# bjzhb666/GS-LoRA

Measured on AMD Instinct MI355X. Metric: forgetting-step images/sec, ViT-P8S8 d6 112px r=8, higher is better.
Workload: dtype fp16

## Files before the change

### gs-lora_amd/gslora_hip/_lib.py

```python
import ctypes as C
import os

import contextlib

_HERE = os.path.dirname(os.path.abspath(__file__))
LIB_PATH = os.environ.get("GSLORA_HIP_LIB") or os.path.join(_HERE, "libgslora_hip.so")
DEV_LIB_PATH = os.path.join(_HERE, "libgslora_hip_dev.so")

F32, BF16, F16 = 0, 1, 2
EPI_STORE, EPI_BIAS_RES_F32, EPI_BIAS_GELU, EPI_MUL, EPI_PATCH, EPI_STORE_F32, EPI_STORE_QKV_HM, EPI_BIAS_RES_BF16, EPI_PATCH_BF16 = 0, 1, 2, 3, 4, 5, 6, 7, 8
EPI_MUL_G8, EPI_BIAS_GELU_G8, EPI_BIAS_RES_F16, EPI_PATCH_F16, EPI_STORE_LN, EPI_STORE_QKV_HM_LN = 9, 10, 11, 12, 13, 14
VERIF_FLIP_SUM, VERIF_PLAIN = 0, 1
U8_NCHW, U8_NHWC = 0, 1
NORM_SPLIT = 8
SEED_ON_DEVICE = 0x80000000

_vp, _i, _l, _f, _d, _u64, _u32 = C.c_void_p, C.c_int, C.c_long, C.c_float, C.c_double, C.c_uint64, C.c_uint32

SIGNATURES = {
    "gsl_version": [],
    "gsl_last_error": [],
    "gsl_patchify": [_vp, _vp, _i, _i, _i, _i, _i, _i, _vp],
    "gsl_unfold_patches": [_vp, _vp, _i, _i, _i, _i, _i, _i, _i, _i, _i, _vp],
    "gsl_patchify_u8": [_vp, _i, _vp, _vp, _i, _i, _i, _i, _i, _i, _vp],
    "gsl_unfold_patches_u8": [_vp, _i, _vp, _vp, _i, _i, _i, _i, _i, _i, _i, _i, _i, _vp],
    "gsl_gemm_nt": [_vp, _i, _vp, _i, _i, _vp, _i, _vp, _i, _i, _i, _i, _i, _i, _f, _vp, _vp, _vp, _vp, _vp, _i,
                    _vp, _vp, _i, _f, _u64, _u32, _vp],
    "gsl_gemm_nt_lora": [_vp, _i, _vp, _i, _i, _vp, _i, _vp, _i, _f, _vp, _i, _i, _i, _i, _i, _vp, _vp, _vp, _vp, _vp, _i,
                         _f, _u64, _u32, _vp],
    "gsl_gemm_mulgrad_ws_elems": [_i, _i, _i],
    "gsl_gemm_nt_lora_mulgrad": [_vp, _i, _vp, _i, _i, _vp, _i, _vp, _i, _f, _vp, _i, _i, _i, _vp, _vp, _i,
                                 _vp, _i, _vp, _l, _l, _vp, _vp, _l, _l, _i, _i, _vp, _i, _f, _i, _vp, _vp],
    "gsl_layernorm_fwd": [_vp, _l, _vp, _vp, _f, _vp, _vp, _vp, _i, _i, _i, _i, _vp],
    "gsl_layernorm_fwd_lora": [_vp, _l, _vp, _vp, _f, _vp, _vp, _vp, _i, _i, _vp, _i, _f, _vp, _vp],
    "gsl_layernorm_bwd": [_vp, _vp, _l, _vp, _vp, _vp, _vp, _vp, _l, _vp, _i, _i, _i, _i, _i, _f, _u64, _u32, _l, _i, _vp, _vp],
    "gsl_attention_fwd": [_vp, _vp, _vp, _i, _i, _i, _f, _i, _i, _vp],
    "gsl_attention_bwd": [_vp, _vp, _vp, _vp, _vp, _vp, _i, _i, _i, _f, _i, _i, _vp],
    "gsl_attention_fwd_cls": [_vp, _vp, _vp, _vp, _i, _i, _i, _f, _i, _i, _vp],
    "gsl_attention_bwd_cls": [_vp, _vp, _vp, _vp, _vp, _vp, _vp, _i, _i, _i, _f, _i, _i, _i, _vp],
    "gsl_lora_grad_ws_elems": [_i, _i, _i],
    "gsl_lora_grad": [_vp, _l, _vp, _i, _vp, _l, _l, _i, _i, _i, _i, _i, _vp, _vp, _vp],
    "gsl_lora_grad_batch_ws_elems": [_vp, _i],
    "gsl_lora_grad_batch": [_vp, _i, _vp, _i, _vp, _vp],
    "gsl_cosface_prep": [_vp, _vp, _i, _i, _vp],
    "gsl_head_fwd": [_vp, _i, _i, _vp, _vp, _f, _vp, _vp, _vp, _vp, _vp, _vp, _i, _i, _i, _f, _f, _vp, _i, _i, _vp],
    "gsl_head_bwd": [_vp, _vp, _vp, _i, _i, _vp, _vp, _vp, _vp, _vp, _vp, _vp, _i, _i, _i, _f, _i, _i, _f, _u64, _u32, _i, _i, _i, _vp, _vp, _i, _vp],
    "gsl_head_fwd_margin": [_vp, _i, _i, _vp, _vp, _f, _vp, _vp, _vp, _vp, _vp, _vp, _i, _i, _i, _f, _f, _vp, _i, _i, _i, _d, _i, _vp, _vp],
    "gsl_head_bwd_margin": [_vp, _vp, _vp, _i, _i, _vp, _vp, _vp, _vp, _vp, _vp, _vp, _i, _i, _i, _f, _i, _i, _f, _u64, _u32, _i, _i, _i, _vp,
                            _vp, _i, _i, _d, _i, _vp, _vp, _vp],
    "gsl_ce_fwd": [_vp, _vp, _vp, _vp, _i, _i, _vp],
    "gsl_ce_bwd": [_vp, _vp, _vp, _f, _vp, _i, _i, _i, _vp],
    "gsl_proto_kl_fwd": [_vp, _vp, _vp, _vp, _vp, _i, _i, _i, _vp],
    "gsl_loss_combine": [_vp, _vp, _vp, _vp, _vp, _vp, _vp, _f, _f, _f, _f, _f, _f, _f, _f, _vp, _vp, _vp, _vp],
    "gsl_loss_combine_pack": [_vp, _vp, _i, _f, _f, _f, _f, _f, _f, _vp, _vp, _vp, _vp],
# ... 69 lines not shown
```

### gs-lora_amd/gslora_hip/build.py

```python
import os
import subprocess
import sys

HERE = os.path.dirname(os.path.abspath(__file__))
CSRC = os.path.join(os.path.dirname(HERE), "csrc")
SOURCES = ["gemm.hip", "norm.hip", "lora.hip", "head.hip", "attention.hip", "verif.hip"]
SOURCES_F16 = ["gemm.hip", "attention.hip"]
HEADERS = ["gsl_common.h", "gsl_h16.h", "exports.map", "gelu_g8_table.inc"]
DEV_ONLY = ["gemm_dev_a.inc", "gemm_dev_b.inc", "gemm_dev_c.inc", "gemm_w4.inc", "gemm_o4.inc"]
OUT = os.path.join(HERE, "libgslora_hip.so")
OUT_DEV = os.path.join(HERE, "libgslora_hip_dev.so")


def needs_build(dev=False):
    out = OUT_DEV if dev else OUT
    if not os.path.exists(out):
        return True
    t = os.path.getmtime(out)
    deps = [os.path.join(CSRC, s) for s in SOURCES + HEADERS + (DEV_ONLY if dev else [])]
    deps.append(os.path.join(os.path.dirname(os.path.dirname(HERE)), "include", "gslora_hip.h"))
    return any(os.path.getmtime(d) > t for d in deps)


def build(force=False, verbose=True, dev=False, defines=(), out=None, tag=None):
# ... 39 lines not shown
```

### gs-lora_amd/gslora_hip/ops.py

```python
import ctypes

import torch

from . import _lib as L

ATTN_MAX_T = 1025


def check_num_tokens(model, T):
    if T > ATTN_MAX_T:
        raise NotImplementedError(f"{model}: this geometry gives {T} tokens per image; the gs-lora_amd attention kernels take at most "
                                  f"{ATTN_MAX_T} (GSL_ATTN_MAX_T: a 32 x 32 patch grid plus the cls token)")


DT = {torch.float32: L.F32, torch.bfloat16: L.BF16, torch.float16: L.F16}


def _p(t):
    return None if t is None else t.data_ptr()


def _stream():
    return torch.cuda.current_stream().cuda_stream

# ... 282 lines not shown
                                           _stream()), "gsl_attention_fwd_cls")
    return o, lse


def attention_bwd_cls(qkv, o, d_o_cls, lse, B, T, H, scale, layout=0, q_cls=None):
    _need(qkv, o, d_o_cls, lse, q_cls)
    nw = 2 if layout == 2 else 3
    dqkv = torch.empty(B * T, nw * H * 64, device=qkv.device, dtype=qkv.dtype)
    dq = torch.empty(B, H * 64, device=qkv.device, dtype=qkv.dtype) if layout == 2 else None
    compact = o.shape[0] == B and lse.dim() == 2
    L.check(L.load().gsl_attention_bwd_cls(_p(qkv), _p(q_cls), _p(o), _p(d_o_cls), _p(lse), _p(dqkv), _p(dq), B, T, H, float(scale),
                                           code(qkv.dtype), int(layout), 1 if compact else 0, _stream()), "gsl_attention_bwd_cls")
    return (dqkv, dq) if layout == 2 else dqkv


_ws_cache = {}
_ws_retired = []


def lora_grad(Y, U, G, gsn, gsj, r, accumulate=True, gscale=None):
    if not (Y.is_cuda and U.is_cuda and Y.stride(1) == 1 and U.stride(1) == 1):
        raise RuntimeError("lora_grad: operands must be CUDA tensors with unit column stride")
    M, N = Y.shape
    lib = L.load()
    need = lib.gsl_lora_grad_ws_elems(M, N, r)
    key = (Y.device.index,)
    ws = _ws_cache.get(key)
    if ws is None or ws.numel() < need:
        if ws is not None:
            _ws_retired.append(ws)
# ... 329 lines not shown
```

### gs-lora_amd/gslora_hip/vit_runner.py

```python
import os

import torch

from . import _lib as L
from . import ops

PADK = 64
OP16 = (torch.bfloat16, torch.float16)
SITE_EMB = 1_000_000
GRAD_STREAM_BF16 = os.environ.get("GSLORA_GRAD_STREAM", "bf16").lower() != "f32"
FWD_STREAM = os.environ.get("GSLORA_FWD_STREAM", "f16").lower()
if FWD_STREAM not in ("f16", "bf16", "f32"):
    raise ValueError(f"GSLORA_FWD_STREAM must be f16, bf16 or f32, not {FWD_STREAM!r}")
GP8 = os.environ.get("GSLORA_GP8", "1") != "0"

FUSE_LORA_GRAD = True
TAIL_CLS = True
QSPLIT = True
INK_MIN_ROWS = 8192
LN1_FOLD = os.environ.get("GSLORA_LN1_FOLD", "1") != "0"
GRAD_TARGET_EXP = int(os.environ.get("GSLORA_GRAD_TARGET_EXP", "0"))
if GRAD_TARGET_EXP and not 4 <= GRAD_TARGET_EXP <= 15:
    raise ValueError(f"GSLORA_GRAD_TARGET_EXP={GRAD_TARGET_EXP}: 0 (default) or 4 .. 15")
INK_SMALL = True
LGRAD_BATCH_MAX_ROWS = 1 << 30
LN_LORA = False
QKV_HEAD_MAJOR = True


class BlockSpec:
    __slots__ = ("ln1", "qkv_w", "qkv_b", "out", "ln2", "l1", "l2", "qkv_lora")

    def __init__(self, ln1, qkv_w, qkv_b, out, ln2, l1, l2, qkv_lora=None):
# ... 173 lines not shown
            self._wcache[key] = ent
        return ent[1]

    def w_conv(self, name, param, dtype):
        def build(p):
            w2 = p.permute(0, 2, 3, 1).reshape(p.shape[0], -1).contiguous()
            return w2 if dtype == torch.float32 else ops.cast(w2, dtype)
        return self._cached(self._wcache, (name, "conv", dtype), param, build)

    def w_kpad(self, name, param, kpad, dtype):
        def build(p):
            w2 = torch.zeros(p.shape[0], kpad, device=p.device, dtype=torch.float32)
            w2[:, :p.shape[1]] = p
            return w2 if dtype == torch.float32 else ops.cast(w2, dtype)
        return self._cached(self._wcache, (name, "kpad", kpad, dtype), param, build)

    def wT(self, name, param, dtype):
        return self._cached(self._wcache, (name, "t", dtype), param, lambda p: ops.transpose_cast(p.contiguous(), dtype))

    PACK_GEOM = {
        "A_rows": lambda R, C, r: (C, 1, r, C, PADK, C),
        "B_cols": lambda R, C, r: (r, 1, R, r, R, PADK),
        "BT_rows": lambda R, C, r: (1, r, r, R, PADK, R),
        "AT_cols": lambda R, C, r: (1, C, C, r, C, PADK),
        "A_rows16": lambda R, C, r: (C, 1, r, C, 16, C),
        "B_cols32": lambda R, C, r: (r, 1, R, r, R, 32),
        "BT_rows16": lambda R, C, r: (1, r, r, R, 16, R),
        "AT_cols32": lambda R, C, r: (1, C, C, r, C, 32),
    }

# ... 150 lines not shown
            pw = self.w_conv("pe", sp.patch_w, dt) if sp.patch_is_conv else self.w("pe", sp.patch_w, dt)
        xbf = dt in OP16 and FWD_STREAM != "f32"
        xf16 = xbf and (FWD_STREAM == "f16" or dt == torch.float16)
        xdt = (torch.float16 if xf16 else torch.bfloat16) if xbf else torch.float32
        epi_res = (L.EPI_BIAS_RES_F16 if xf16 else L.EPI_BIAS_RES_BF16) if xbf else L.EPI_BIAS_RES_F32
        x = torch.empty(M, D, device=img.device, dtype=xdt)
        ops.gemm_nt(patches, pw, x, epilogue=(L.EPI_PATCH_F16 if xf16 else L.EPI_PATCH_BF16) if xbf else L.EPI_PATCH, bias=sp.patch_b.detach(),
                    pos=sp.pos.detach()[0, :T].contiguous(), cls=sp.cls.detach().reshape(-1), T=T,
                    p_drop=p_emb, seed=seed, site=SITE_EMB | sflag)
        del patches
        stash = []
        for i, blk in enumerate(sp.blocks):
            n1, n2 = blk.ln1, blk.ln2
            attn_lora_live = attn_site and not blk.qkv_lora.merged
            fold = LN1_FOLD and dt in OP16 and x.dtype == dt and not attn_lora_live
            if fold:
                mean1, rstd1 = ops.layernorm_stats(x, D, M, D, n1.weight.detach(), n1.bias.detach(), eps, dt)
                xn = None
            else:
                xn, mean1, rstd1 = ops.layernorm_fwd(x, D, M, D, n1.weight.detach(), n1.bias.detach(), eps, dt)
            tail = TAIL_CLS and i == len(sp.blocks) - 1 and sp.pool == "cls"
            qsplit = tail and QSPLIT and not attn_site
            inner = H * 64
            hm = 1 if (QKV_HEAD_MAJOR and dt in OP16) else 0
            epi_qkv = L.EPI_STORE_QKV_HM if hm else L.EPI_STORE
            uq = q_cls = None
            if qsplit and fold:
                wf, cq, dq_ = self.w_ln(f"qkv{i}", blk.qkv_w, n1.weight, n1.bias, blk.qkv_b, dt)
                qkv = torch.empty(M, 2 * inner, device=img.device, dtype=dt)
                ops.gemm_nt(x, wf[inner:], qkv, epilogue=L.EPI_STORE_LN, pos=mean1, cls=rstd1, aux=cq[inner:], bias=dq_[inner:])
                q_cls = torch.empty(B, inner, device=img.device, dtype=dt)
                ops.gemm_nt(x.view(B, T * D)[:, :D], wf[:inner], q_cls, epilogue=L.EPI_STORE_LN, T=T, pos=mean1, cls=rstd1,
                            aux=cq[:inner], bias=dq_[:inner])
                hm = 2
            elif qsplit:
                wq = self.w(f"qkv{i}", blk.qkv_w, dt)
                qb_ = None if blk.qkv_b is None else blk.qkv_b.detach()
                qkv = torch.empty(M, 2 * inner, device=img.device, dtype=dt)
                ops.gemm_nt(xn, wq[inner:], qkv, bias=None if qb_ is None else qb_[inner:])
                q_cls = torch.empty(B, inner, device=img.device, dtype=dt)
                ops.gemm_nt(xn.view(B, T * D)[:, :D], wq[:inner], q_cls, bias=None if qb_ is None else qb_[:inner].contiguous())
                hm = 2
# ... 2 lines not shown
                qo = self.qkv_lora_ops(i, blk.qkv_lora, dt)
                uq = torch.empty(M, PADK, device=img.device, dtype=dt)
                ops.gemm_nt(xn, qo["A_rows"], uq, alpha=s_lora)
                ops.gemm_nt(xn, self.w(f"qkv{i}", blk.qkv_w, dt), qkv, A2=uq, W2=qo["Bblk"], epilogue=epi_qkv, T=T,
                            bias=None if blk.qkv_b is None else blk.qkv_b.detach())
            elif fold:
                wf, cq, dq_ = self.w_ln(f"qkv{i}", blk.qkv_w, n1.weight, n1.bias, blk.qkv_b, dt)
                qkv = torch.empty(M, 3 * inner, device=img.device, dtype=dt)
                ops.gemm_nt(x, wf, qkv, epilogue=L.EPI_STORE_QKV_HM_LN if hm else L.EPI_STORE_LN, T=T, pos=mean1, cls=rstd1, aux=cq, bias=dq_)
            else:
                qkv = torch.empty(M, 3 * inner, device=img.device, dtype=dt)
                ops.gemm_nt(xn, self.w(f"qkv{i}", blk.qkv_w, dt), qkv, epilogue=epi_qkv, T=T,
                            bias=None if blk.qkv_b is None else blk.qkv_b.detach())
            xn_keep = xn if (attn_site and save) else None
            del xn
            if tail:
                o, lse = ops.attention_fwd_cls(qkv, B, T, H, sp.attn_scale, layout=hm, q_cls=q_cls)
                xres, Mr = x.view(B, T, D)[:, 0].contiguous(), B
            else:
                o, lse = ops.attention_fwd(qkv, B, T, H, sp.attn_scale, layout=hm)
                xres, Mr = x, M
            x1 = torch.empty(Mr, D, device=img.device, dtype=xdt)
            ops.gemm_nt(o, self.w(f"wo{i}", blk.out.weight, dt), x1, epilogue=epi_res,
                        bias=blk.out.bias.detach(), res=xres, p_drop=p_drop, seed=seed, site=(4 * i) | sflag)
            del xres
            l1, l2 = blk.l1, blk.l2
            mlp = l1.weight.shape[0]
            lora_on = r > 0 and not attn_site and not l1.merged
            ln_u1 = LN_LORA and lora_on and r <= 16 and D in (512, 768) and x1.dtype == torch.bfloat16 and dt == torch.bfloat16
            if ln_u1:
                xn2, mean2, rstd2, u1_ln = ops.layernorm_fwd_lora(x1, D, Mr, D, n2.weight.detach(), n2.bias.detach(), eps,
# ... 29 lines not shown
                    ops.gemm_nt(h, self.lora_pack(f"A2_{i}", l2.lora_A, "A_rows", dt), u2, alpha=s_lora)
            else:
                ops.gemm_nt(xn2, self.w(f"w1_{i}", l1.weight, dt), h, epilogue=epi_gelu, bias=l1.bias.detach(),
                            out2=gp, p_drop=p_drop, seed=seed, site=(4 * i + 1) | sflag)
            x2 = torch.empty(Mr, D, device=img.device, dtype=xdt)
            if lora_on and self.lora_in_kernel(dt, Mr, D):
                ops.gemm_nt_lora(h, self.w(f"w2_{i}", l2.weight, dt), self.lora_pack(f"A2_{i}", l2.lora_A, "A_rows16", dt),
                                 self.lora_pack(f"B2_{i}", l2.lora_B, "B_cols32", dt), s_lora, u2, x2, epilogue=epi_res,
                                 bias=l2.bias.detach(), res=x1, p_drop=p_drop, seed=seed, site=(4 * i + 2) | sflag)
            else:
                ops.gemm_nt(h, self.w(f"w2_{i}", l2.weight, dt), x2, epilogue=epi_res, A2=u2,
                            W2=self.lora_pack(f"B2_{i}", l2.lora_B, "B_cols", dt) if lora_on else None,
                            bias=l2.bias.detach(), res=x1, p_drop=p_drop, seed=seed, site=(4 * i + 2) | sflag)
            if save:
                stash.append(dict(x=x, mean1=mean1, rstd1=rstd1, qkv=qkv, qkv_hm=hm, o=o, lse=lse, x1=x1, mean2=mean2, rstd2=rstd2,
                                  xn2=xn2, u1=u1, u1c=u1c, h=h, gp=gp, u2=u2, lora_on=lora_on, xn=xn_keep, uq=uq, tail=tail, q_cls=q_cls))
            x = x2
        hn = sp.final_ln
        Th = x.shape[0] // B
        cos_y = None
        if linear_head:
            Wn = sp.head_w.detach().contiguous() if (sp.head_kind == "linear" or label is not None) else None
            logits, emb, meanh, rstdh = ops.head_fwd(x, B, Th, D, hn.weight.detach(), hn.bias.detach(), eps, Wn, None, 1.0, 0.0,
                                                     head_bias=sp.head_b.detach(), linear=Wn is not None, pool_mean=(sp.pool == "mean"))
        else:
            if label is None:
                Wn = None
            elif sp.head_w.requires_grad:
                Wn = ops.cosface_prep(sp.head_w.detach().contiguous())
            else:
                Wn = self._cached(self._wcache, ("cosface_wn",), sp.head_w, lambda p: ops.cosface_prep(p.contiguous()))
# ... 123 lines not shown
                dxn2 = torch.empty(Mrows, D, device=dev, dtype=dt)
                ops.gemm_nt(da, self.wT(f"w1_{i}", l1.weight, dt), dxn2, A2=v1,
                            W2=self.lora_pack(f"A1_{i}", l1.lora_A, "AT_cols", dt))
            del da, v1, v2
            n2 = blk.ln2
            if sparse and not tail:
                dx1, dx1b = ops.layernorm_bwd(dxn2, st["x1"], T * D, n2.weight.detach(), cls_rows(st["mean2"].view(-1, 1), 1).view(-1),
                                              cls_rows(st["rstd2"].view(-1, 1), 1).view(-1), dx,
                                              p_drop=p_drop, seed=seed, site=(4 * i) | sflag, drop_row_stride=T * D, gmax=gmax)
            else:
                dx1, dx1b = ops.layernorm_bwd(dxn2, st["x1"], D, n2.weight.detach(), st["mean2"], st["rstd2"], dx,
                                              p_drop=p_drop, seed=seed, site=(4 * i) | sflag, gmax=gmax)
            del dxn2
            d_o = torch.empty(Mrows, H * 64, device=dev, dtype=dt)
            ops.gemm_nt(dx1b, self.wT(f"wo{i}", blk.out.weight, dt), d_o)
            dxn1 = torch.empty(B * T, D, device=dev, dtype=dt)
            if sparse and st["q_cls"] is not None:
                inner = H * 64
                dkv, dq_cls = ops.attention_bwd_cls(st["qkv"], st["o"], d_o, st["lse"], B, T, H, sp.attn_scale, layout=2, q_cls=st["q_cls"])
                wt = self.wT(f"qkv{i}", blk.qkv_w, dt)
                ops.gemm_nt(dkv, wt[:, inner:], dxn1)
                rows = dxn1.view(B, T * D)[:, :D]
                ops.gemm_nt(dq_cls, wt[:, :inner], rows, epilogue={torch.bfloat16: L.EPI_BIAS_RES_BF16, torch.float16: L.EPI_BIAS_RES_F16}.get(dt, L.EPI_BIAS_RES_F32),
                            bias=self._zeros(D, dev), res=rows)
                del dkv, dq_cls
            else:
                if sparse:
                    dqkv = ops.attention_bwd_cls(st["qkv"], st["o"], d_o, st["lse"], B, T, H, sp.attn_scale, layout=st["qkv_hm"])
                else:
                    dqkv = ops.attention_bwd(st["qkv"], st["o"], d_o, st["lse"], B, T, H, sp.attn_scale, layout=st["qkv_hm"])
                ops.gemm_nt(dqkv, self.wT(f"qkv{i}", blk.qkv_w, dt), dxn1)
                del dqkv
            del d_o, dx1b
            n1 = blk.ln1
            dx, dxb = ops.layernorm_bwd(dxn1, st["x"], D, n1.weight.detach(), st["mean1"], st["rstd1"], dx1,
                                        p_drop=p_drop, seed=seed, site=(4 * (i - 1) + 2) | sflag,
                                        dres_cls_T=T if sparse else 0, gmax=gmax)
            saved["layers"][i] = None
        if not torch.cuda.is_current_stream_capturing():
            self.build_pack_tables(dt)

# ... 85 lines not shown
```

### include/gslora_hip.h

```cpp
#ifndef GSLORA_HIP_H
#define GSLORA_HIP_H

#include <stdint.h>

#ifdef __cplusplus
extern "C" {
#endif

#define GSL_API __attribute__((visibility("default")))

typedef void* gsl_stream_t;

enum gsl_dtype { GSL_F32 = 0, GSL_BF16 = 1, GSL_F16 = 2 };

enum gsl_status {
  GSL_OK = 0,
  GSL_ERR_ARG = -1,
  GSL_ERR_LAUNCH = -2,
  GSL_ERR_UNSUPPORTED = -3
};

enum gsl_epilogue {
  GSL_EPI_STORE = 0,
  GSL_EPI_BIAS_RES_F32 = 1,
// ... 55 lines not shown
                           float* mean, float* rstd, int M, int D, const void* P, int ldp, float alpha, void* u, gsl_stream_t s);
GSL_API int gsl_layernorm_bwd(const void* dy, const void* x, long x_row_stride, const float* gamma,
                      const float* mean, const float* rstd, const void* dres,
                      void* dx, long io_row_stride, void* dxb, int M, int D, int dtype, int stream_dtype, int x_dtype,
                      float p_drop, uint64_t seed, uint32_t site, long drop_row_stride, int dres_cls_T, float* gmax, gsl_stream_t s);

#define GSL_ATTN_MAX_T 1025
GSL_API int gsl_attention_fwd(const void* qkv, void* o, float* lse, int B, int T, int H, float scale, int dtype, int qkv_layout, gsl_stream_t s);
GSL_API int gsl_attention_bwd(const void* qkv, const void* o, const void* d_o, const float* lse, void* dqkv,
                      float* delta_ws, int B, int T, int H, float scale, int dtype, int qkv_layout, gsl_stream_t s);
GSL_API int gsl_attention_fwd_cls(const void* qkv, const void* q_cls, void* o_cls, float* lse_cls, int B, int T, int H, float scale,
                                  int dtype, int qkv_layout, gsl_stream_t s);
GSL_API int gsl_attention_bwd_cls(const void* qkv, const void* q_cls, const void* o, const void* d_o_cls, const float* lse, void* dqkv,
                                  void* dq_cls, int B, int T, int H, float scale, int dtype, int qkv_layout, int cls_compact, gsl_stream_t s);

GSL_API long gsl_lora_grad_ws_elems(int M, int N, int r);
GSL_API int gsl_lora_grad(const void* Y, long ldy, const void* U, int ldu, float* G, long gsn, long gsj,
                  int M, int N, int r, int dtype, int accumulate, float* ws, const float* gscale, gsl_stream_t s);
typedef struct gsl_lgrad_desc {
  const void* Y; long ldy; const void* U; int ldu; int M; int N; int r; int accumulate; int pad_; float* G; long gsn, gsj;
} gsl_lgrad_desc;
GSL_API long gsl_lora_grad_batch_ws_elems(const gsl_lgrad_desc* descs, int n);
GSL_API int gsl_lora_grad_batch(const gsl_lgrad_desc* descs, int n, float* ws, int dtype, const float* gscale, gsl_stream_t s);


GSL_API int gsl_cosface_prep(const float* W, float* Wn, int C, int D, gsl_stream_t s);
GSL_API int gsl_head_fwd(const void* x, int x_dtype, int T, const float* gamma, const float* beta, float eps,
                 const float* Wn, const int64_t* label, float* emb, float* mean, float* rstd,
                 float* logits, int B, int D, int C, float cos_s, float cos_m,
                 const float* head_bias, int linear_head, int pool_mean, gsl_stream_t s);
// ... 77 lines not shown
```

Before: 45890.

## Stream last-block CLS attention through LN rows with folded K/V weights

For the final block, where only the CLS query matters, the K and V projections over all tokens are no longer computed. The CLS query is multiplied into block-diagonal folded K weights, and a new kernel scores LayerNorm-ed rows held in registers, applies softmax, and pools the normalized rows into per-head averages. A small GEMM with the folded V/O weights then produces the output, and a mirror backward kernel produces gradients for x-normalized and qt. This drops the large T×2·inner QKV GEMM and attention for the tail block in exchange for H·D-sized intermediates and new kernels with shape limits.

```diff
diff --git a/gs-lora_amd/csrc/cls_stream.hip b/gs-lora_amd/csrc/cls_stream.hip
--- /dev/null
+++ b/gs-lora_amd/csrc/cls_stream.hip
@@ -0,0 +1,451 @@
+#include "gsl_common.h"
+
+using namespace gsl;
+
+namespace {
+
+constexpr int CS_WAVES = 16;
+constexpr int CS_R = 13;
+constexpr int CS_TMAX = CS_WAVES * CS_R;
+constexpr int CS_HMAX = 16;
+constexpr int CS_RED = 8;
+
+__device__ __forceinline__ constexpr int cs_lane_of(int j) { return ((j & 1) << 5) | (((j >> 1) & 1) << 4) | (((j >> 2) & 1) << 3) | (((j >> 3) & 1) << 2); }
+__device__ __forceinline__ int cs_slot_of(int lane) { return ((lane >> 5) & 1) | (((lane >> 4) & 1) << 1) | (((lane >> 3) & 1) << 2) | (((lane >> 2) & 1) << 3); }
+__device__ __forceinline__ float cs_pair(float a0, float a1, int lane) {
+  const bool up = (lane & 32) != 0;
+  return (up ? a1 : a0) + __shfl_xor(up ? a0 : a1, 32, 64);
+}
+__device__ __forceinline__ float cs_sum8(float (&v)[8], int lane) {
+#pragma unroll
+  for (int n = 8, m = 16; n > 1; n >>= 1, m >>= 1) {
+    const bool up = (lane & m) != 0;
+#pragma unroll
+    for (int k = 0; k < n / 2; ++k) {
+      const float keep = up ? v[2 * k + 1] : v[2 * k], send = up ? v[2 * k] : v[2 * k + 1];
+      v[k] = keep + __shfl_xor(send, m, 64);
+    }
+  }
+  v[0] += __shfl_xor(v[0], 2, 64);
+  v[0] += __shfl_xor(v[0], 1, 64);
+  return v[0];
+}
+__device__ __forceinline__ float cs_bcast(float v, int src_lane) {
+  return __int_as_float(__builtin_amdgcn_readlane(__float_as_int(v), src_lane));
+}
+
+template <bool XF16>
+__device__ __forceinline__ void cs_unpack4(const uint2 u, float f[4]) {
+  if constexpr (XF16) { unpack2h(u.x, f[0], f[1]); unpack2h(u.y, f[2], f[3]); }
+  else {
+    f[0] = __uint_as_float(u.x << 16); f[1] = __uint_as_float(u.x & 0xffff0000u);
+    f[2] = __uint_as_float(u.y << 16); f[3] = __uint_as_float(u.y & 0xffff0000u);
+  }
+}
+
+template <int NC>
+__device__ __forceinline__ void cs_load_vec(const float* __restrict__ p, int lane, float (&v)[NC][4]) {
+#pragma unroll
+  for (int c = 0; c < NC; ++c) Elem<float>::ld4(p + (c * 64 + lane) * 4, v[c]);
+}
+
+template <int NC, bool HOLD>
+struct CsRows {
+  static constexpr int D = 256 * NC;
+  uint2 xr[HOLD ? CS_R : 1][NC];
+  const uint16_t* base;
+  int T, w, lane;
+  __device__ __forceinline__ void fetch(int r, uint2 (&row)[NC]) const {
+    const int t = r * CS_WAVES + w, tc = t < T ? t : T - 1;
+#pragma unroll
+    for (int c = 0; c < NC; ++c) {
+      const uint2 v = *reinterpret_cast<const uint2*>(base + (size_t)tc * D + c * 256 + lane * 4);
+      row[c] = make_uint2(t < T ? v.x : 0u, t < T ? v.y : 0u);
+    }
+  }
+  __device__ __forceinline__ void init(const uint16_t* __restrict__ x, int b, int T_, int w_, int lane_) {
+    base = x + (size_t)b * T_ * D; T = T_; w = w_; lane = lane_;
+    if constexpr (HOLD) {
+#pragma unroll
+      for (int r = 0; r < CS_R; ++r) fetch(r, xr[r]);
+    }
+  }
+  __device__ __forceinline__ void pin() {
+    if constexpr (HOLD) {
+#pragma unroll
+      for (int r = 0; r < CS_R; ++r)
+#pragma unroll
+        for (int c = 0; c < NC; ++c) asm volatile("" : "+v"(xr[r][c].x), "+v"(xr[r][c].y));
+    } else asm volatile("" : "+s"(base));
+  }
+  __device__ __forceinline__ void get(int r, uint2 (&row)[NC]) const {
+    if constexpr (HOLD) {
+#pragma unroll
+      for (int c = 0; c < NC; ++c) row[c] = xr[r][c];
+    } else fetch(r, row);
+  }
+  __device__ __forceinline__ void get(int r, uint2 (&row)[NC]) {
+    if constexpr (!HOLD) asm volatile("" : "+s"(base));
+    static_cast<const CsRows*>(this)->get(r, row);
+  }
+};
+
+template <int NC, bool XF16>
+__device__ __forceinline__ float cs_row_dot(const uint2 (&row)[NC], const float (&g)[NC][4]) {
+  float a = 0.f;
+#pragma unroll
+  for (int c = 0; c < NC; ++c) {
+    float f[4];
+    cs_unpack4<XF16>(row[c], f);
+#pragma unroll
+    for (int i = 0; i < 4; ++i) a = fmaf(g[c][i], f[i], a);
+  }
+  return a;
+}
+template <int NC, bool XF16, bool HOLD>
+__device__ __forceinline__ float cs_row_dots(CsRows<NC, HOLD>& X, const float (&g)[NC][4], int lane) {
+  X.pin();
+  float v[8];
+#pragma unroll
+  for (int k = 0; k < 8; ++k) {
+    float a[2] = {0.f, 0.f};
+#pragma unroll
+    for (int j = 0; j < 2; ++j) {
+      if (2 * k + j < CS_R) {
+        uint2 row[NC];
+        X.get(2 * k + j, row);
+        a[j] = cs_row_dot<NC, XF16>(row, g);
+      }
+    }
+    v[k] = cs_pair(a[0], a[1], lane);
+  }
+  return cs_sum8(v, lane);
+}
+
+template <int NC, bool XF16, bool HOLD>
+__device__ __forceinline__ void cs_pool(CsRows<NC, HOLD>& X, const float* __restrict__ wgt, const float (&mu)[CS_R], const float (&rs)[CS_R],
+                                        float* __restrict__ red, int w, int lane, float& tot0, float& tot1) {
+  constexpr int D = 256 * NC;
+  float acc[NC][4];
+#pragma unroll
+  for (int c = 0; c < NC; ++c)
+#pragma unroll
+    for (int i = 0; i < 4; ++i) acc[c][i] = 0.f;
+  float ms = 0.f;
+  X.pin();
+#pragma unroll
+  for (int r = 0; r < CS_R; ++r) {
+    const float wr = wgt[r * CS_WAVES + w] * rs[r];
+    ms = fmaf(wr, mu[r], ms);
+    uint2 row[NC];
+    X.get(r, row);
+#pragma unroll
+    for (int c = 0; c < NC; ++c) {
+      float f[4];
+      cs_unpack4<XF16>(row[c], f);
+#pragma unroll
+      for (int i = 0; i < 4; ++i) acc[c][i] = fmaf(wr, f[i], acc[c][i]);
+    }
+  }
+#pragma unroll
+  for (int c = 0; c < NC; ++c)
+#pragma unroll
+    for (int i = 0; i < 4; ++i) acc[c][i] -= ms;
+  if (w >= CS_RED) {
+#pragma unroll
+    for (int c = 0; c < NC; ++c) Elem<float>::st4(red + (w - CS_RED) * D + (c * 64 + lane) * 4, acc[c]);
+  }
+  __syncthreads();
+  if (w < CS_RED) {
+#pragma unroll
+    for (int c = 0; c < NC; ++c) {
+      float o[4];
+      Elem<float>::ld4(red + w * D + (c * 64 + lane) * 4, o);
+#pragma unroll
+      for (int i = 0; i < 4; ++i) o[i] = acc[c][i] + o[i];
+      Elem<float>::st4(red + w * D + (c * 64 + lane) * 4, o);
+    }
+  }
+  __syncthreads();
+  tot0 = tot1 = 0.f;
+  const int tid = threadIdx.x;
+  if (tid < D / 2) {
+#pragma unroll
+    for (int k = 0; k < CS_RED; ++k) {
+      const float2 v = *reinterpret_cast<const float2*>(red + k * D + 2 * tid);
+      tot0 += v.x; tot1 += v.y;
+    }
+  }
+  __syncthreads();
+}
+
+template <int NC, bool XF16>
+__global__ __launch_bounds__(CS_WAVES * 64) void cls_stream_fwd_kernel(const uint16_t* __restrict__ x, const float* __restrict__ gamma,
+                                                                       const float* __restrict__ beta, float eps, const float* __restrict__ qt,
+                                                                       float scale, uint16_t* __restrict__ xbar, int o_f16, float* __restrict__ p_out,
+                                                                       float* __restrict__ mean, float* __restrict__ rstd, int T, int H) {
+  fp16_sat_on();
+  constexpr int D = 256 * NC;
+  __shared__ float sm_p[CS_HMAX * CS_TMAX];
+  __shared__ float red[CS_RED * D];
+  const int b = blockIdx.x, tid = threadIdx.x, lane = tid & 63, w = __builtin_amdgcn_readfirstlane(tid >> 6);
+  constexpr bool HOLD = NC <= 2;
+  CsRows<NC, HOLD> X;
+  X.init(x, b, T, w, lane);
+  for (int i = tid; i < H * CS_TMAX; i += CS_WAVES * 64) sm_p[i] = 0.f;
+
+  const int slot = cs_slot_of(lane), my_t = slot * CS_WAVES + w;
+  const bool mine = (lane & 3) == 0 && slot < CS_R && my_t < T;
+  float my_mu, my_rs, mu[CS_R], rs[CS_R];
+  {
+    float v[8];
+#pragma unroll
+    for (int k = 0; k < 8; ++k) {
+      float s2[2] = {0.f, 0.f};
+#pragma unroll
+      for (int j = 0; j < 2; ++j) {
+        if (2 * k + j < CS_R) {
+          uint2 row[NC];
+          X.get(2 * k + j, row);
+#pragma unroll
+          for (int c = 0; c < NC; ++c) {
+            float f[4];
+            cs_unpack4<XF16>(row[c], f);
+#pragma unroll
+            for (int i = 0; i < 4; ++i) s2[j] += f[i];
+          }
+        }
+      }
+      v[k] = cs_pair(s2[0], s2[1], lane);
+    }
+    my_mu = cs_sum8(v, lane) * (1.0f / D);
+#pragma unroll
+    for (int r = 0; r < CS_R; ++r) mu[r] = cs_bcast(my_mu, cs_lane_of(r));
+    X.pin();
+#pragma unroll
+    for (int k = 0; k < 8; ++k) {
+      float q2[2] = {0.f, 0.f};
+#pragma unroll
+      for (int j = 0; j < 2; ++j) {
+        if (2 * k + j < CS_R) {
+          uint2 row[NC];
+          X.get(2 * k + j, row);
+#pragma unroll
+          for (int c = 0; c < NC; ++c) {
+            float f[4];
+            cs_unpack4<XF16>(row[c], f);
+#pragma unroll
+            for (int i = 0; i < 4; ++i) { f[i] -= mu[2 * k + j]; q2[j] = __fadd_rn(q2[j], __fmul_rn(f[i], f[i])); }
+          }
+        }
+      }
+      v[k] = cs_pair(q2[0], q2[1], lane);
+    }
+    my_rs = rsqrtf(fmaf(cs_sum8(v, lane), 1.0f / D, eps));
+#pragma unroll
+    for (int r = 0; r < CS_R; ++r) rs[r] = cs_bcast(my_rs, cs_lane_of(r));
+    if (mine) { mean[(size_t)b * T + my_t] = my_mu; rstd[(size_t)b * T + my_t] = my_rs; }
+  }
+  __syncthreads();
+
+  for (int h = 0; h < H; ++h) {
+    float g[NC][4], ga[NC][4];
+    cs_load_vec<NC>(qt + ((size_t)b * H + h) * D, lane, g);
+    cs_load_vec<NC>(gamma, lane, ga);
+    float c1 = 0.f;
+#pragma unroll
+    for (int c = 0; c < NC; ++c)
+#pragma unroll
+      for (int i = 0; i < 4; ++i) { g[c][i] *= ga[c][i]; c1 += g[c][i]; }
+    c1 = wave_sum(c1);
+    const float tot = cs_row_dots<NC, XF16, HOLD>(X, g, lane);
+    if (mine) sm_p[h * CS_TMAX + my_t] = scale * my_rs * (tot - my_mu * c1);
+  }
+  __syncthreads();
+
+  for (int h = w; h < H; h += CS_WAVES) {
+    float v[4], m = -3.0e38f;
+#pragma unroll
+    for (int k = 0; k < 4; ++k) {
+      const int t = lane + 64 * k;
+      v[k] = (t < T) ? sm_p[h * CS_TMAX + t] : -3.0e38f;
+      m = fmaxf(m, v[k]);
+    }
+    m = wave_max(m);
+    float e = 0.f;
+#pragma unroll
+    for (int k = 0; k < 4; ++k) {
+      const int t = lane + 64 * k;
+      v[k] = (t < T) ? expf(v[k] - m) : 0.f;
+      e += v[k];
+    }
+    e = wave_sum(e);
+#pragma unroll
+    for (int k = 0; k < 4; ++k) {
+      const int t = lane + 64 * k;
+      if (t < T) {
+        const float p = v[k] / e;
+        sm_p[h * CS_TMAX + t] = p;
+        p_out[((size_t)b * H + h) * T + t] = p;
+      }
+    }
+  }
+  __syncthreads();
+
+  for (int h = 0; h < H; ++h) {
+    float t0, t1;
+    cs_pool<NC, XF16, HOLD>(X, sm_p + h * CS_TMAX, mu, rs, red, w, lane, t0, t1);
+    if (tid < D / 2) {
+      const float2 ga = *reinterpret_cast<const float2*>(gamma + 2 * tid), be = *reinterpret_cast<const float2*>(beta + 2 * tid);
+      *reinterpret_cast<uint32_t*>(xbar + ((size_t)b * H + h) * D + 2 * tid) = pack2s(fmaf(ga.x, t0, be.x), fmaf(ga.y, t1, be.y), o_f16);
+    }
+  }
+}
+
+template <int NC, bool XF16>
+__global__ __launch_bounds__(CS_WAVES * 64) void cls_stream_bwd_kernel(const uint16_t* __restrict__ x, const float* __restrict__ gamma,
+                                                                       const float* __restrict__ mean, const float* __restrict__ rstd,
+                                                                       const float* __restrict__ qt, const float* __restrict__ dxbar,
+                                                                       const float* __restrict__ p_in, float scale, uint16_t* __restrict__ dxn,
+                                                                       uint16_t* __restrict__ dqt, int o_f16, int T, int H) {
+  fp16_sat_on();
+  constexpr int D = 256 * NC;
+  constexpr int RC = (NC == 3) ? 3 : 4;
+  __shared__ float sm_p[CS_HMAX * CS_TMAX];
+  __shared__ float sm_ds[CS_HMAX * CS_TMAX];
+  __shared__ float red[CS_RED * D];
+  const int b = blockIdx.x, tid = threadIdx.x, lane = tid & 63, w = __builtin_amdgcn_readfirstlane(tid >> 6);
+  constexpr bool HOLD = NC <= 2;
+  CsRows<NC, HOLD> X;
+  X.init(x, b, T, w, lane);
+  for (int i = tid; i < H * CS_TMAX; i += CS_WAVES * 64) { sm_p[i] = 0.f; sm_ds[i] = 0.f; }
+  const int slot = cs_slot_of(lane), my_t = slot * CS_WAVES + w;
+  const bool mine = (lane & 3) == 0 && slot < CS_R && my_t < T;
+  const bool have = slot < CS_R && my_t < T;
+  const float my_mu = have ? mean[(size_t)b * T + my_t] : 0.f, my_rs = have ? rstd[(size_t)b * T + my_t] : 0.f;
+  __syncthreads();
+
+  for (int h = 0; h < H; ++h) {
+    float g[NC][4], ga[NC][4];
+    cs_load_vec<NC>(dxbar + ((size_t)b * H + h) * D, lane, g);
+    cs_load_vec<NC>(gamma, lane, ga);
+    float c1 = 0.f;
+#pragma unroll
+    for (int c = 0; c < NC; ++c)
+#pragma unroll
+      for (int i = 0; i < 4; ++i) { g[c][i] *= ga[c][i]; c1 += g[c][i]; }
+    c1 = wave_sum(c1);
+    const float tot = cs_row_dots<NC, XF16, HOLD>(X, g, lane);
+    if (mine) sm_ds[h * CS_TMAX + my_t] = my_rs * (tot - my_mu * c1);
+  }
+  __syncthreads();
+
+  for (int h = w; h < H; h += CS_WAVES) {
+    float p[4], dp[4], dot = 0.f;
+#pragma unroll
+    for (int k = 0; k < 4; ++k) {
+      const int t = lane + 64 * k;
+      p[k] = (t < T) ? p_in[((size_t)b * H + h) * T + t] : 0.f;
+      dp[k] = (t < T) ? sm_ds[h * CS_TMAX + t] : 0.f;
+      dot = fmaf(p[k], dp[k], dot);
+    }
+    dot = wave_sum(dot);
+#pragma unroll
+    for (int k = 0; k < 4; ++k) {
+      const int t = lane + 64 * k;
+      if (t < T) { sm_p[h * CS_TMAX + t] = p[k]; sm_ds[h * CS_TMAX + t] = p[k] * (dp[k] - dot); }
+    }
+  }
+  __syncthreads();
+
+  float mu[CS_R], rs[CS_R];
+#pragma unroll
+  for (int r = 0; r < CS_R; ++r) { mu[r] = cs_bcast(my_mu, cs_lane_of(r)); rs[r] = cs_bcast(my_rs, cs_lane_of(r)); }
+  for (int h = 0; h < H; ++h) {
+    float t0, t1;
+    cs_pool<NC, XF16, HOLD>(X, sm_ds + h * CS_TMAX, mu, rs, red, w, lane, t0, t1);
+    if (tid < D / 2) {
+      const float2 ga = *reinterpret_cast<const float2*>(gamma + 2 * tid);
+      *reinterpret_cast<uint32_t*>(dqt + ((size_t)b * H + h) * D + 2 * tid) = pack2s(scale * ga.x * t0, scale * ga.y * t1, o_f16);
+    }
+  }
+
+#pragma unroll
+  for (int r0 = 0; r0 < CS_R; r0 += RC) {
+    float acc[RC][NC][4];
+#pragma unroll
+    for (int r = 0; r < RC; ++r)
+#pragma unroll
+      for (int c = 0; c < NC; ++c)
+#pragma unroll
+        for (int i = 0; i < 4; ++i) acc[r][c][i] = 0.f;
+    for (int h = 0; h < H; ++h) {
+      float dv[NC][4], qv[NC][4];
+      cs_load_vec<NC>(dxbar + ((size_t)b * H + h) * D, lane, dv);
+      cs_load_vec<NC>(qt + ((size_t)b * H + h) * D, lane, qv);
+#pragma unroll
+      for (int r = 0; r < RC; ++r) {
+        if (r0 + r < CS_R) {
+          const float pw = sm_p[h * CS_TMAX + (r0 + r) * CS_WAVES + w], dw = scale * sm_ds[h * CS_TMAX + (r0 + r) * CS_WAVES + w];
+#pragma unroll
+          for (int c = 0; c < NC; ++c)
+#pragma unroll
+            for (int i = 0; i < 4; ++i) acc[r][c][i] = fmaf(dw, qv[c][i], fmaf(pw, dv[c][i], acc[r][c][i]));
+        }
+      }
+    }
+#pragma unroll
+    for (int r = 0; r < RC; ++r) {
+      const int t = (r0 + r) * CS_WAVES + w;
+      if (r0 + r < CS_R && t < T) {
+#pragma unroll
+        for (int c = 0; c < NC; ++c)
+          *reinterpret_cast<uint2*>(dxn + ((size_t)b * T + t) * D + c * 256 + lane * 4) =
+              make_uint2(pack2s(acc[r][c][0], acc[r][c][1], o_f16), pack2s(acc[r][c][2], acc[r][c][3], o_f16));
+      }
+    }
+  }
+}
+
+}
+
+#define GSL_CS_DISPATCH(KERNEL, ...)                                                                                         \
+  do {                                                                                                                       \
+    const dim3 grid(B), blk(CS_WAVES * 64);                                                                                  \
+    const bool xf16 = x_dtype == GSL_F16;                                                                                    \
+    if (D == 256 && xf16) hipLaunchKernelGGL((KERNEL<1, true>), grid, blk, 0, as_stream(s), __VA_ARGS__);                    \
+    else if (D == 256) hipLaunchKernelGGL((KERNEL<1, false>), grid, blk, 0, as_stream(s), __VA_ARGS__);                      \
+    else if (D == 512 && xf16) hipLaunchKernelGGL((KERNEL<2, true>), grid, blk, 0, as_stream(s), __VA_ARGS__);               \
+    else if (D == 512) hipLaunchKernelGGL((KERNEL<2, false>), grid, blk, 0, as_stream(s), __VA_ARGS__);                      \
+    else if (xf16) hipLaunchKernelGGL((KERNEL<3, true>), grid, blk, 0, as_stream(s), __VA_ARGS__);                           \
+    else hipLaunchKernelGGL((KERNEL<3, false>), grid, blk, 0, as_stream(s), __VA_ARGS__);                                    \
+  } while (0)
+
+#define GSL_CS_CHECK_SHAPE()                                                                                                         \
+  GSL_CHECK_ARG(B > 0 && T > 1 && T <= GSL_CLS_STREAM_MAX_T, "1 < T <= GSL_CLS_STREAM_MAX_T (208: the rows of an image live in registers)"); \
+  GSL_CHECK_ARG(H > 0 && H <= GSL_CLS_STREAM_MAX_H, "1 <= H <= GSL_CLS_STREAM_MAX_H (16)");                                            \
+  GSL_CHECK_ARG(D == 256 || D == 512 || D == 768, "D: 256, 512 or 768");                                                             \
+  GSL_CHECK_ARG(dtype == GSL_BF16 || dtype == GSL_F16, "dtype: a 16-bit operand format");                                            \
+  GSL_CHECK_ARG((x_dtype == GSL_BF16 && dtype == GSL_BF16) || x_dtype == GSL_F16, "x dtype: a 16-bit stream (bf16 only with bf16 operands)")
+
+static_assert(GSL_CLS_STREAM_MAX_T == CS_TMAX && GSL_CLS_STREAM_MAX_H == CS_HMAX, "header limits");
+
+extern "C" int gsl_cls_stream_attn_fwd(const void* x, const float* gamma, const float* beta, float eps, const float* qt, float scale,
+                                       void* xbar, float* p, float* mean, float* rstd, int B, int T, int H, int D, int dtype, int x_dtype,
+                                       gsl_stream_t s) {
+  GSL_CHECK_ARG(x && gamma && beta && qt && xbar && p && mean && rstd, "null");
+  GSL_CS_CHECK_SHAPE();
+  const int o_f16 = dtype == GSL_F16;
+  GSL_CS_DISPATCH(cls_stream_fwd_kernel, (const uint16_t*)x, gamma, beta, eps, qt, scale, (uint16_t*)xbar, o_f16, p, mean, rstd, T, H);
+  return check_launch("gsl_cls_stream_attn_fwd");
+}
+
+extern "C" int gsl_cls_stream_attn_bwd(const void* x, const float* gamma, const float* mean, const float* rstd, const float* qt,
+                                       const float* dxbar, const float* p, float scale, void* dxn, void* dqt, int B, int T, int H, int D,
+                                       int dtype, int x_dtype, gsl_stream_t s) {
+  GSL_CHECK_ARG(x && gamma && mean && rstd && qt && dxbar && p && dxn && dqt, "null");
+  GSL_CS_CHECK_SHAPE();
+  const int o_f16 = dtype == GSL_F16;
+  GSL_CS_DISPATCH(cls_stream_bwd_kernel, (const uint16_t*)x, gamma, mean, rstd, qt, dxbar, p, scale, (uint16_t*)dxn, (uint16_t*)dqt, o_f16, T, H);
+  return check_launch("gsl_cls_stream_attn_bwd");
+}
diff --git a/gs-lora_amd/gslora_hip/_lib.py b/gs-lora_amd/gslora_hip/_lib.py
--- a/gs-lora_amd/gslora_hip/_lib.py
+++ b/gs-lora_amd/gslora_hip/_lib.py
@@ -38,6 +38,8 @@
     "gsl_attention_bwd": [_vp, _vp, _vp, _vp, _vp, _vp, _i, _i, _i, _f, _i, _i, _vp],
     "gsl_attention_fwd_cls": [_vp, _vp, _vp, _vp, _i, _i, _i, _f, _i, _i, _vp],
     "gsl_attention_bwd_cls": [_vp, _vp, _vp, _vp, _vp, _vp, _vp, _i, _i, _i, _f, _i, _i, _i, _vp],
+    "gsl_cls_stream_attn_fwd": [_vp, _vp, _vp, _f, _vp, _f, _vp, _vp, _vp, _vp, _i, _i, _i, _i, _i, _i, _vp],
+    "gsl_cls_stream_attn_bwd": [_vp, _vp, _vp, _vp, _vp, _vp, _vp, _f, _vp, _vp, _i, _i, _i, _i, _i, _i, _vp],
     "gsl_lora_grad_ws_elems": [_i, _i, _i],
     "gsl_lora_grad": [_vp, _l, _vp, _i, _vp, _l, _l, _i, _i, _i, _i, _i, _vp, _vp, _vp],
     "gsl_lora_grad_batch_ws_elems": [_vp, _i],
diff --git a/gs-lora_amd/gslora_hip/build.py b/gs-lora_amd/gslora_hip/build.py
--- a/gs-lora_amd/gslora_hip/build.py
+++ b/gs-lora_amd/gslora_hip/build.py
@@ -4,7 +4,7 @@
 
 HERE = os.path.dirname(os.path.abspath(__file__))
 CSRC = os.path.join(os.path.dirname(HERE), "csrc")
-SOURCES = ["gemm.hip", "norm.hip", "lora.hip", "head.hip", "attention.hip", "verif.hip"]
+SOURCES = ["gemm.hip", "norm.hip", "lora.hip", "head.hip", "attention.hip", "cls_stream.hip", "verif.hip"]
 SOURCES_F16 = ["gemm.hip", "attention.hip"]
 HEADERS = ["gsl_common.h", "gsl_h16.h", "exports.map", "gelu_g8_table.inc"]
 DEV_ONLY = ["gemm_dev_a.inc", "gemm_dev_b.inc", "gemm_dev_c.inc", "gemm_w4.inc", "gemm_o4.inc"]
diff --git a/gs-lora_amd/gslora_hip/ops.py b/gs-lora_amd/gslora_hip/ops.py
--- a/gs-lora_amd/gslora_hip/ops.py
+++ b/gs-lora_amd/gslora_hip/ops.py
@@ -320,6 +320,38 @@
     return (dqkv, dq) if layout == 2 else dqkv
 
 
+CLS_STREAM_MAX_T, CLS_STREAM_MAX_H, CLS_STREAM_DIMS = 208, 16, (256, 512, 768)
+
+
+def cls_stream_ok(T, H, D, dtype, x_dtype):
+    return (2 <= T <= CLS_STREAM_MAX_T and H <= CLS_STREAM_MAX_H and D in CLS_STREAM_DIMS and dtype in (torch.bfloat16, torch.float16)
+            and (x_dtype == torch.float16 or (x_dtype == torch.bfloat16 and dtype == torch.bfloat16)))
+
+
+@_profiled("attn_fwd_cls_stream", lambda x, gamma, beta, eps, qt, B, T, H, *a, **k: (B * T, x.shape[1], T, H))
+def cls_stream_attn_fwd(x, gamma, beta, eps, qt, B, T, H, scale, dtype):
+    _need(x, gamma, beta, qt)
+    D = x.shape[1]
+    xbar = torch.empty(B, H * D, device=x.device, dtype=dtype)
+    p = torch.empty(B, H, T, device=x.device, dtype=torch.float32)
+    mean = torch.empty(B * T, device=x.device, dtype=torch.float32)
+    rstd = torch.empty(B * T, device=x.device, dtype=torch.float32)
+    L.check(L.load().gsl_cls_stream_attn_fwd(_p(x), _p(gamma), _p(beta), float(eps), _p(qt), float(scale), _p(xbar), _p(p), _p(mean), _p(rstd),
+                                             B, T, H, D, code(dtype), code(x.dtype), _stream()), "gsl_cls_stream_attn_fwd")
+    return xbar, p, mean, rstd
+
+
+@_profiled("attn_bwd_cls_stream", lambda x, gamma, mean, rstd, qt, dxbar, p, B, T, H, *a, **k: (B * T, x.shape[1], T, H))
+def cls_stream_attn_bwd(x, gamma, mean, rstd, qt, dxbar, p, B, T, H, scale, dtype):
+    _need(x, gamma, mean, rstd, qt, dxbar, p)
+    D = x.shape[1]
+    dxn = torch.empty(B * T, D, device=x.device, dtype=dtype)
+    dqt = torch.empty(B, H * D, device=x.device, dtype=dtype)
+    L.check(L.load().gsl_cls_stream_attn_bwd(_p(x), _p(gamma), _p(mean), _p(rstd), _p(qt), _p(dxbar), _p(p), float(scale), _p(dxn), _p(dqt),
+                                             B, T, H, D, code(dtype), code(x.dtype), _stream()), "gsl_cls_stream_attn_bwd")
+    return dxn, dqt
+
+
 _ws_cache = {}
 _ws_retired = []
 
diff --git a/gs-lora_amd/gslora_hip/vit_runner.py b/gs-lora_amd/gslora_hip/vit_runner.py
--- a/gs-lora_amd/gslora_hip/vit_runner.py
+++ b/gs-lora_amd/gslora_hip/vit_runner.py
@@ -17,6 +17,7 @@
 FUSE_LORA_GRAD = True
 TAIL_CLS = True
 QSPLIT = True
+CLS_STREAM = os.environ.get("GSLORA_CLS_STREAM", "1") != "0"
 INK_MIN_ROWS = 8192
 LN1_FOLD = os.environ.get("GSLORA_LN1_FOLD", "1") != "0"
 GRAD_TARGET_EXP = int(os.environ.get("GSLORA_GRAD_TARGET_EXP", "0"))
@@ -220,6 +221,16 @@
             w2[:, :p.shape[1]] = p
             return w2 if dtype == torch.float32 else ops.cast(w2, dtype)
         return self._cached(self._wcache, (name, "kpad", kpad, dtype), param, build)
+
+    def w_cls_stream(self, name, qkv_w, H, dtype):
+        def build(p):
+            inner, D = H * 64, p.shape[1]
+            wk, wv = p[inner:2 * inner].float().view(H, 64, D), p[2 * inner:].float().view(H, 64, D)
+            kq = torch.block_diag(*[wk[h].t() for h in range(H)])
+            vo = torch.block_diag(*[wv[h] for h in range(H)])
+            c = lambda t: ops.cast(t.contiguous(), dtype)
+            return dict(kq=c(kq), vo=c(vo), vd=c(vo.t()), kd=c(kq.t()))
+        return self._cached(self._wcache, (name, "clsbd", dtype), qkv_w, build)
 
     def wT(self, name, param, dtype):
         return self._cached(self._wcache, (name, "t", dtype), param, lambda p: ops.transpose_cast(p.contiguous(), dtype))
@@ -400,18 +411,35 @@
             n1, n2 = blk.ln1, blk.ln2
             attn_lora_live = attn_site and not blk.qkv_lora.merged
             fold = LN1_FOLD and dt in OP16 and x.dtype == dt and not attn_lora_live
-            if fold:
+            tail = TAIL_CLS and i == len(sp.blocks) - 1 and sp.pool == "cls"
+            qsplit = tail and QSPLIT and not attn_site
+            stream = qsplit and CLS_STREAM and ops.cls_stream_ok(T, H, D, dt, x.dtype)
+            if stream:
+                xn, mean1, rstd1 = ops.layernorm_fwd(x, T * D, B, D, n1.weight.detach(), n1.bias.detach(), eps, dt)
+            elif fold:
                 mean1, rstd1 = ops.layernorm_stats(x, D, M, D, n1.weight.detach(), n1.bias.detach(), eps, dt)
                 xn = None
             else:
                 xn, mean1, rstd1 = ops.layernorm_fwd(x, D, M, D, n1.weight.detach(), n1.bias.detach(), eps, dt)
-            tail = TAIL_CLS and i == len(sp.blocks) - 1 and sp.pool == "cls"
-            qsplit = tail and QSPLIT and not attn_site
             inner = H * 64
             hm = 1 if (QKV_HEAD_MAJOR and dt in OP16) else 0
             epi_qkv = L.EPI_STORE_QKV_HM if hm else L.EPI_STORE
-            uq = q_cls = None
-            if qsplit and fold:
+            uq = q_cls = cs = None
+            if stream:
+                wq = self.w(f"qkv{i}", blk.qkv_w, dt)
+                qb_ = None if blk.qkv_b is None else blk.qkv_b.detach()
+                bd = self.w_cls_stream(f"qkv{i}", blk.qkv_w, H, dt)
+                q_cls = torch.empty(B, inner, device=img.device, dtype=dt)
+                ops.gemm_nt(xn, wq[:inner], q_cls, bias=None if qb_ is None else qb_[:inner].contiguous())
+                qt = torch.empty(B, H * D, device=img.device, dtype=torch.float32)
+                ops.gemm_nt(q_cls, bd["kq"], qt, epilogue=L.EPI_STORE_F32)
+                xbar, p_cls, mean1, rstd1 = ops.cls_stream_attn_fwd(x, n1.weight.detach(), n1.bias.detach(), eps, qt, B, T, H, sp.attn_scale, dt)
+                o = torch.empty(B, inner, device=img.device, dtype=dt)
+                ops.gemm_nt(xbar, bd["vo"], o, bias=None if qb_ is None else qb_[2 * inner:].contiguous())
+                qkv = lse = None
+                cs = dict(qt=qt, p=p_cls, bd=bd)
+                del xbar
+            elif qsplit and fold:
                 wf, cq, dq_ = self.w_ln(f"qkv{i}", blk.qkv_w, n1.weight, n1.bias, blk.qkv_b, dt)
                 qkv = torch.empty(M, 2 * inner, device=img.device, dtype=dt)
                 ops.gemm_nt(x, wf[inner:], qkv, epilogue=L.EPI_STORE_LN, pos=mean1, cls=rstd1, aux=cq[inner:], bias=dq_[inner:])
@@ -444,7 +472,9 @@
                             bias=None if blk.qkv_b is None else blk.qkv_b.detach())
             xn_keep = xn if (attn_site and save) else None
             del xn
-            if tail:
+            if stream:
+                xres, Mr = x.view(B, T, D)[:, 0].contiguous(), B
+            elif tail:
                 o, lse = ops.attention_fwd_cls(qkv, B, T, H, sp.attn_scale, layout=hm, q_cls=q_cls)
                 xres, Mr = x.view(B, T, D)[:, 0].contiguous(), B
             else:
@@ -504,7 +534,7 @@
                             bias=l2.bias.detach(), res=x1, p_drop=p_drop, seed=seed, site=(4 * i + 2) | sflag)
             if save:
                 stash.append(dict(x=x, mean1=mean1, rstd1=rstd1, qkv=qkv, qkv_hm=hm, o=o, lse=lse, x1=x1, mean2=mean2, rstd2=rstd2,
-                                  xn2=xn2, u1=u1, u1c=u1c, h=h, gp=gp, u2=u2, lora_on=lora_on, xn=xn_keep, uq=uq, tail=tail, q_cls=q_cls))
+                                  xn2=xn2, u1=u1, u1c=u1c, h=h, gp=gp, u2=u2, lora_on=lora_on, xn=xn_keep, uq=uq, tail=tail, q_cls=q_cls, cs=cs))
             x = x2
         hn = sp.final_ln
         Th = x.shape[0] // B
@@ -658,9 +688,22 @@
             del dxn2
             d_o = torch.empty(Mrows, H * 64, device=dev, dtype=dt)
             ops.gemm_nt(dx1b, self.wT(f"wo{i}", blk.out.weight, dt), d_o)
-            dxn1 = torch.empty(B * T, D, device=dev, dtype=dt)
-            if sparse and st["q_cls"] is not None:
+            if sparse and st["cs"] is not None:
+                inner, cs = H * 64, st["cs"]
+                dxbar = torch.empty(B, H * D, device=dev, dtype=torch.float32)
+                ops.gemm_nt(d_o, cs["bd"]["vd"], dxbar, epilogue=L.EPI_STORE_F32)
+                dxn1, dqt = ops.cls_stream_attn_bwd(st["x"], blk.ln1.weight.detach(), st["mean1"], st["rstd1"], cs["qt"], dxbar, cs["p"],
+                                                    B, T, H, sp.attn_scale, dt)
+                dq_cls = torch.empty(B, inner, device=dev, dtype=dt)
+                ops.gemm_nt(dqt, cs["bd"]["kd"], dq_cls)
+                wt = self.wT(f"qkv{i}", blk.qkv_w, dt)
+                rows = dxn1.view(B, T * D)[:, :D]
+                ops.gemm_nt(dq_cls, wt[:, :inner], rows, epilogue={torch.bfloat16: L.EPI_BIAS_RES_BF16, torch.float16: L.EPI_BIAS_RES_F16}[dt],
+                            bias=self._zeros(D, dev), res=rows)
+                del dxbar, dqt, dq_cls
+            elif sparse and st["q_cls"] is not None:
                 inner = H * 64
+                dxn1 = torch.empty(B * T, D, device=dev, dtype=dt)
                 dkv, dq_cls = ops.attention_bwd_cls(st["qkv"], st["o"], d_o, st["lse"], B, T, H, sp.attn_scale, layout=2, q_cls=st["q_cls"])
                 wt = self.wT(f"qkv{i}", blk.qkv_w, dt)
                 ops.gemm_nt(dkv, wt[:, inner:], dxn1)
@@ -669,6 +712,7 @@
                             bias=self._zeros(D, dev), res=rows)
                 del dkv, dq_cls
             else:
+                dxn1 = torch.empty(B * T, D, device=dev, dtype=dt)
                 if sparse:
                     dqkv = ops.attention_bwd_cls(st["qkv"], st["o"], d_o, st["lse"], B, T, H, sp.attn_scale, layout=st["qkv_hm"])
                 else:
diff --git a/include/gslora_hip.h b/include/gslora_hip.h
--- a/include/gslora_hip.h
+++ b/include/gslora_hip.h
@@ -93,6 +93,15 @@
 GSL_API int gsl_attention_bwd_cls(const void* qkv, const void* q_cls, const void* o, const void* d_o_cls, const float* lse, void* dqkv,
                                   void* dq_cls, int B, int T, int H, float scale, int dtype, int qkv_layout, int cls_compact, gsl_stream_t s);
 
+#define GSL_CLS_STREAM_MAX_T 208
+#define GSL_CLS_STREAM_MAX_H 16
+GSL_API int gsl_cls_stream_attn_fwd(const void* x, const float* gamma, const float* beta, float eps, const float* qt, float scale,
+                                    void* xbar, float* p, float* mean, float* rstd, int B, int T, int H, int D, int dtype, int x_dtype,
+                                    gsl_stream_t s);
+GSL_API int gsl_cls_stream_attn_bwd(const void* x, const float* gamma, const float* mean, const float* rstd, const float* qt,
+                                    const float* dxbar, const float* p, float scale, void* dxn, void* dqt, int B, int T, int H, int D,
+                                    int dtype, int x_dtype, gsl_stream_t s);
+
 GSL_API long gsl_lora_grad_ws_elems(int M, int N, int r);
 GSL_API int gsl_lora_grad(const void* Y, long ldy, const void* U, int ldu, float* G, long gsn, long gsj,
                   int M, int N, int r, int dtype, int accumulate, float* ws, const float* gscale, gsl_stream_t s);
```

Result: no change. 46260 (median of 6 runs) (+0.8%).
